# EdoardoLuciani/ARayTracingJourney

Measured on AMD Instinct MI355X. Metric: Mray/s (primary+shadow), Sponza-class 1080p, higher is better.
Workload: dtype f32; 1 GPU; sponza_like(seed=0x5A0A, 262816 triangles, 25 primitives) 1920x1080, 1 light(s), 794216 shadow rays/frame; width=1920, height=1080, lights=1, parallelism=single GPU, 8 frames in flight

## Files before the change

araytracingjourney_amd/csrc/art_trace.hip:

```cpp
#include "art_internal.h"
#include <type_traits>

namespace art {

struct V3 { float x, y, z; };
__device__ __forceinline__ V3 mk(float x, float y, float z) { V3 r; r.x = x; r.y = y; r.z = z; return r; }
__device__ __forceinline__ V3 operator+(V3 a, V3 b) { return mk(a.x + b.x, a.y + b.y, a.z + b.z); }
__device__ __forceinline__ V3 operator-(V3 a, V3 b) { return mk(a.x - b.x, a.y - b.y, a.z - b.z); }
__device__ __forceinline__ V3 operator*(V3 a, V3 b) { return mk(a.x * b.x, a.y * b.y, a.z * b.z); }
__device__ __forceinline__ V3 operator*(V3 a, float s) { return mk(a.x * s, a.y * s, a.z * s); }
__device__ __forceinline__ V3 neg(V3 a) { return mk(-a.x, -a.y, -a.z); }
__device__ __forceinline__ float dot3(V3 a, V3 b) { return fmaf(a.z, b.z, fmaf(a.y, b.y, a.x * b.x)); }
__device__ __forceinline__ V3 cross3(V3 a, V3 b) {
    return mk(fmaf(a.y, b.z, -(a.z * b.y)), fmaf(a.z, b.x, -(a.x * b.z)), fmaf(a.x, b.y, -(a.y * b.x)));
}
constexpr float kExactLo = 0x1p-96f, kExactHi = 0x1p96f;
__device__ __forceinline__ float sqrt_core(float x) {
    float s = __builtin_amdgcn_sqrtf(x);
    float dn = __uint_as_float(__float_as_uint(s) - 1u), up = __uint_as_float(__float_as_uint(s) + 1u);
    float vp = fmaf(-dn, s, x), vs = fmaf(-up, s, x);
    s = vp <= 0.0f ? dn : s;
    return vs > 0.0f ? up : s;
}
__device__ __forceinline__ float rcp_core(float d) {
// ... 128 lines not shown
    float tf = fminf(fminf(fmaxf(t0x, t1x), fmaxf(t0y, t1y)), fmaxf(t0z, t1z));
    return fmaxf(tn, r.tmin) <= fminf(tf, tlimit);
}
#define ART_BARY_EPS 1.0e-6f
__device__ __forceinline__ bool moller_trumbore(const Ray &r, V3 v0, V3 e1, V3 e2, float &t, float &u, float &v) {
    V3 p = cross3(r.d, e2);
    float det = dot3(e1, p);
    if (det == 0.0f) return false;
    float inv = 1.0f / det;
    V3 tv = r.o - v0;
    float uu = dot3(tv, p) * inv;
    if (!(uu >= -ART_BARY_EPS && uu <= 1.0f + ART_BARY_EPS)) return false;
    V3 q = cross3(tv, e1);
    float vv = dot3(r.d, q) * inv;
    if (!(vv >= -ART_BARY_EPS && uu + vv <= 1.0f + ART_BARY_EPS)) return false;
    float tt = dot3(e2, q) * inv;
    if (!(tt > r.tmin && tt < r.tmax)) return false;
    t = tt; u = uu; v = vv;
    return true;
}

__device__ __forceinline__ bool moller_trumbore_flat(const Ray &r, V3 v0, V3 e1, V3 e2, float &t, float &u, float &v) {
    V3 p = cross3(r.d, e2);
    float det = dot3(e1, p);
    float inv = 1.0f / det;
    V3 tv = r.o - v0;
    u = dot3(tv, p) * inv;
    V3 q = cross3(tv, e1);
    v = dot3(r.d, q) * inv;
    t = dot3(e2, q) * inv;
    return (det != 0.0f) & (u >= -ART_BARY_EPS) & (u <= 1.0f + ART_BARY_EPS) & (v >= -ART_BARY_EPS) & (u + v <= 1.0f + ART_BARY_EPS) & (t > r.tmin) & (t < r.tmax);
}

constexpr int kLdsStack = 16;
constexpr int kOvfStack = 80;
constexpr int kBlock = 256;
constexpr int kFrameBlock = 64;
constexpr int kTraceBlock = 64;
struct Tune { uint32_t chunk, refill, blocks, leaf_batch; };
static const Tune kPreset[4] = {{64, 12, 1536, 1}, {128, 24, 1024, 1}, {256, 16, 2048, 8}, {1024, 24, 2048, 8}};
static Tune tune_over(Tune t, const TraceTune &o) {
    if (o.chunk >= 64 && o.chunk <= 65536) t.chunk = o.chunk;
    if (o.refill >= 1 && o.refill <= 64) t.refill = o.refill;
    if (o.blocks >= 1 && o.blocks <= 16384) t.blocks = o.blocks;
    if (o.leaf_batch >= 1 && o.leaf_batch <= 64) t.leaf_batch = o.leaf_batch;
    return t;
}
static Tune tune(bool pipelined, bool ao, const TraceTune &o) { return tune_over(kPreset[(ao ? 2 : 0) + (pipelined ? 1 : 0)], o); }
constexpr int kCursorStride = 32;

__device__ __forceinline__ bool local_to_xy(uint32_t p, const uint32_t *__restrict__ tile_list, uint32_t tiles_x, uint32_t W, uint32_t H, uint32_t &x, uint32_t &y) {
    uint32_t tile = tile_list[p >> 10];
    uint32_t q = p & 1023u, sub = q >> 6, l = q & 63u;
    x = (tile % tiles_x) * kTile + (sub & 3u) * 8u + (l & 7u);
    y = (tile / tiles_x) * kTile + (sub >> 2) * 8u + (l >> 3);
    return x < W && y < H;
}

constexpr int kOvfStack4 = 288;
template <bool ANY, int OVF, int LDSN = kLdsStack, bool ALPHA = false> struct TravBase {
    Ray r;
    float tbest, bu, bv;
    uint32_t bpos, bgid;
    int cur, sp;
    __device__ __forceinline__ void start(V3 o, V3 d, float tmin, float tmax) {
        ray_init(r, o, d, tmin, tmax);
// ... 68 lines not shown
        const bool ngx = r.inv.x < 0.0f, ngy = r.inv.y < 0.0f, ngz = r.inv.z < 0.0f;
        const uint32_t nxw = ngx ? b.w : b.x, fxw = ngx ? b.x : b.w, nyw = ngy ? c.x : b.y, fyw = ngy ? b.y : c.x, nzw = ngz ? c.y : b.z, fzw = ngz ? b.z : c.y;
        const float lim = this->tbest;
#pragma unroll
        for (int i = 0; i < 4; i++) {
            float tnx = fmaf(fmaf((float)((nxw >> (8 * i)) & 255u), sx, ox), r.inv.x, -r.ood.x), tfx = fmaf(fmaf((float)((fxw >> (8 * i)) & 255u), sx, ox), r.inv.x, -r.ood.x);
            float tny = fmaf(fmaf((float)((nyw >> (8 * i)) & 255u), sy, oy), r.inv.y, -r.ood.y), tfy = fmaf(fmaf((float)((fyw >> (8 * i)) & 255u), sy, oy), r.inv.y, -r.ood.y);
            float tnz = fmaf(fmaf((float)((nzw >> (8 * i)) & 255u), sz, oz), r.inv.z, -r.ood.z), tfz = fmaf(fmaf((float)((fzw >> (8 * i)) & 255u), sz, oz), r.inv.z, -r.ood.z);
            float tn = fmaxf(fmaxf(tnx, tny), tnz), tf = fminf(fminf(tfx, tfy), tfz);
            te[i] = tn;
            h[i] = fmaxf(tn, r.tmin) <= fminf(tf, lim);
        }
        float tn = 3.0e38f; int ni = -1;
        if (ANY) {
#pragma unroll
            for (int i = 3; i >= 0; i--) if (h[i]) ni = i;
        } else
#pragma unroll
        for (int i = 0; i < 4; i++) if (h[i] && te[i] < tn) { tn = te[i]; ni = i; }
        if (ni < 0) return this->pop(lds, ovf);
#pragma unroll
        for (int i = 0; i < 4; i++) if (h[i] && i != ni) this->push(refs[i], lds, ovf);
        this->cur = ni == 0 ? refs[0] : (ni == 1 ? refs[1] : (ni == 2 ? refs[2] : refs[3]));
        return false;
    }
};

constexpr int kPacketStack = 288;
__device__ __forceinline__ bool ao_slot_decode(uint32_t slot, uint32_t spp, uint32_t &p, uint32_t &j);
__device__ __forceinline__ V3 ao_dir(V3 N, float tx, float ty, float tz);

__device__ __forceinline__ void ao_ray(const CameraArg &cam, uint32_t W, uint32_t H, uint32_t x, uint32_t y, float depth, float4 nm, uint32_t smp, V3 &o, V3 &d);

__device__ __forceinline__ uint64_t ballot64(bool p) { return __builtin_amdgcn_ballot_w64(p); }

typedef float f4v __attribute__((ext_vector_type(4)));
__device__ __forceinline__ void st_nt(float4 *p, float4 v) { __builtin_nontemporal_store(f4v{v.x, v.y, v.z, v.w}, reinterpret_cast<f4v *>(p)); }
__device__ __forceinline__ void st_nt(float *p, float v) { __builtin_nontemporal_store(v, p); }
typedef float f3v __attribute__((ext_vector_type(3)));
__device__ __forceinline__ void st_nt_rgb(float4 *tiles, size_t texel, float4 v) { __builtin_nontemporal_store(f3v{v.x, v.y, v.z}, reinterpret_cast<f3v *>(reinterpret_cast<float *>(tiles) + 3 * texel)); }
__device__ __forceinline__ float4 ld_nt(const float4 *p) { f4v v = __builtin_nontemporal_load(reinterpret_cast<const f4v *>(p)); return make_float4(v.x, v.y, v.z, v.w); }

template <int OCT> __device__ __forceinline__ bool slab_oct(const Ray &r, float lx, float ly, float lz, float hx, float hy, float hz, float tlimit, float &tn) {
    if (OCT >= 8) return slab(r, lx, ly, lz, hx, hy, hz, tlimit, tn);
    float nx = fmaf((OCT & 1) ? hx : lx, r.inv.x, -r.ood.x), fx = fmaf((OCT & 1) ? lx : hx, r.inv.x, -r.ood.x);
    float ny = fmaf((OCT & 2) ? hy : ly, r.inv.y, -r.ood.y), fy = fmaf((OCT & 2) ? ly : hy, r.inv.y, -r.ood.y);
    float nz = fmaf((OCT & 4) ? hz : lz, r.inv.z, -r.ood.z), fz = fmaf((OCT & 4) ? lz : hz, r.inv.z, -r.ood.z);
    tn = fmaxf(fmaxf(nx, ny), nz);
    float tf = fminf(fminf(fx, fy), fz);
    return fmaxf(tn, r.tmin) <= fminf(tf, tlimit);
}

struct ConstQuads {
    typedef float Quad __attribute__((ext_vector_type(4)));
    __attribute__((address_space(4))) const Quad *p;
    __device__ __forceinline__ float4 operator[](int i) const { Quad v = p[i]; return make_float4(v.x, v.y, v.z, v.w); }
};
template <class T> __device__ __forceinline__ ConstQuads const_quads(const T *p) { ConstQuads q; q.p = (__attribute__((address_space(4))) const ConstQuads::Quad *)(uintptr_t)p; return q; }

#ifdef ART_PACKET_PROF
__device__ unsigned long long g_packet_prof[24];
#define PPROF(i, n) do { if ((threadIdx.x & 63u) == 0) atomicAdd(&g_packet_prof[(ANY ? 12 : 0) + (i)], (unsigned long long)(n)); } while (0)
#else
#define PPROF(i, n)
#endif
struct PacketHints { int cur, sp; uint32_t n; };
__device__ __forceinline__ PacketHints hints_seed(int *stk, uint32_t w0, uint32_t w1, uint32_t w2, uint32_t w3, uint32_t n_leaves) {
    PacketHints h{0, 0, 0u};
    if ((w0 & w1 & w2 & w3) == kHintEmpty) return h;
    const bool lane0 = (threadIdx.x & 63u) == 0;
    if (w3 < n_leaves) { if (lane0) stk[h.sp] = h.cur; h.sp++; h.cur = (int)~w3; }
    if (w2 < n_leaves) { if (lane0) stk[h.sp] = h.cur; h.sp++; h.cur = (int)~w2; }
    if (w1 < n_leaves) { if (lane0) stk[h.sp] = h.cur; h.sp++; h.cur = (int)~w1; }
    if (w0 < n_leaves) { if (lane0) stk[h.sp] = h.cur; h.sp++; h.cur = (int)~w0; }
    return h;
}
template <bool ANY, bool WIDE, int OCT, bool COUNT = false, bool ALPHA = false, bool HINTS = false>
__device__ __forceinline__ void packet_walk(const FrameArgs &a, const Ray &r, bool &on, int *stk, float &tbest, float &bu, float &bv, uint32_t &bpos, uint32_t &bgid, uint32_t &steps, PacketHints &h) {
    int cur = HINTS ? h.cur : 0, sp = HINTS ? h.sp : 0;
    constexpr int kPop = kAbsentChild;
    const auto cull = [&]() -> uint32_t { return ANY ? (a.ray_masks >> 8) & 0xFFu : a.ray_masks & 0xFFu; };
    if (ALPHA && cull() == 0u) return;
#ifdef ART_PACKET_PROF
    unsigned long long pp_[12] = {1, 0, 0, 0, 0, 0, 0, OCT == 8, 0, 0, 0, 0}; bool from_stack_ = false; int hints_left_ = 0;
#endif
#ifdef ART_PACKET_PROF
    if (HINTS) hints_left_ = sp;
#endif
    for (;;) {
#ifdef ART_PACKET_PROF
        const unsigned long long tk0_ = __builtin_amdgcn_s_memtime(); const bool was_node_ = cur >= 0;
#endif
        if (COUNT) steps++;
        if (cur >= 0 && WIDE) {
            ConstQuads nq = const_quads(a.widef + cur);
            float4 w0 = nq[0], w1 = nq[1], w2 = nq[2], w3 = nq[3], w4 = nq[4], w5 = nq[5], w6 = nq[6], w7 = nq[7];
            const int c0 = __float_as_int(w6.x), c1 = __float_as_int(w6.y), c2 = __float_as_int(w6.z), c3 = __float_as_int(w6.w);
            float te;
            const uint64_t m0 = ballot64(slab_oct<OCT>(r, w0.x, w0.y, w0.z, w0.w, w1.x, w1.y, tbest, te));
            const uint64_t m1 = ballot64(slab_oct<OCT>(r, w1.z, w1.w, w2.x, w2.y, w2.z, w2.w, tbest, te));
            const uint64_t m2 = ballot64(slab_oct<OCT>(r, w3.x, w3.y, w3.z, w3.w, w4.x, w4.y, tbest, te));
            const uint64_t m3 = ballot64(slab_oct<OCT>(r, w4.z, w4.w, w5.x, w5.y, w5.z, w5.w, tbest, te));
#ifdef ART_PACKET_PROF
            pp_[1]++; pp_[6] += (m0 != 0ull) + (m1 != 0ull) + (m2 != 0ull) + (m3 != 0ull); from_stack_ = false;
#endif
            const uint32_t ax = __float_as_uint(w7.y);
            const bool rev = OCT < 8 ? ((OCT >> ax) & 1) != 0 : 2 * (int)__popcll(ballot64(on && (ax == 0 ? r.inv.x : (ax == 1 ? r.inv.y : r.inv.z)) < 0.0f)) > (int)__popcll(ballot64(on));
            const bool lane0 = (threadIdx.x & 63u) == 0;
            int next = kPop;
            if (!rev) {
                if (m3 != 0ull) next = c3;
                if (m2 != 0ull) { if (next != kPop) { if (lane0) stk[min(sp, kPacketStack - 1)] = next; sp = min(sp + 1, kPacketStack); } next = c2; }
                if (m1 != 0ull) { if (next != kPop) { if (lane0) stk[min(sp, kPacketStack - 1)] = next; sp = min(sp + 1, kPacketStack); } next = c1; }
                if (m0 != 0ull) { if (next != kPop) { if (lane0) stk[min(sp, kPacketStack - 1)] = next; sp = min(sp + 1, kPacketStack); } next = c0; }
            } else {
                if (m0 != 0ull) next = c0;
                if (m1 != 0ull) { if (next != kPop) { if (lane0) stk[min(sp, kPacketStack - 1)] = next; sp = min(sp + 1, kPacketStack); } next = c1; }
                if (m2 != 0ull) { if (next != kPop) { if (lane0) stk[min(sp, kPacketStack - 1)] = next; sp = min(sp + 1, kPacketStack); } next = c2; }
                if (m3 != 0ull) { if (next != kPop) { if (lane0) stk[min(sp, kPacketStack - 1)] = next; sp = min(sp + 1, kPacketStack); } next = c3; }
            }
            cur = next;
        } else if (cur >= 0) {
            ConstQuads nq = const_quads(a.nodes + cur);
            float4 q0 = nq[0], q1 = nq[1], q2 = nq[2], q3 = nq[3];
            int c0 = __float_as_int(q3.x), c1 = __float_as_int(q3.y);
            float te0, te1;
            uint64_t m0 = ballot64(slab_oct<OCT>(r, q0.x, q0.y, q0.z, q0.w, q1.x, q1.y, tbest, te0));
            uint64_t m1 = ballot64(slab_oct<OCT>(r, q1.z, q1.w, q2.x, q2.y, q2.z, q2.w, tbest, te1));
            if (m0 != 0ull && m1 != 0ull) {
                uint64_t fl = ballot64(te0 <= te1), both = m0 & m1;
                uint64_t f0 = (m0 & ~m1) | (both & fl), f1 = (m1 & ~m0) | (both & ~fl);
                bool first0 = (int)__popcll(f0) >= (int)__popcll(f1);
                if ((threadIdx.x & 63u) == 0) stk[min(sp, kPacketStack - 1)] = first0 ? c1 : c0;
                sp = min(sp + 1, kPacketStack);
                cur = first0 ? c0 : c1;
            } else if (m0 != 0ull) cur = c0;
            else if (m1 != 0ull) cur = c1;
            else cur = kPop;
        } else {
            uint32_t pos = (uint32_t)~cur;
            typedef __attribute__((address_space(4))) const uint32_t *Words;
            bool unseen = false;
            const auto flagged = [&]() -> bool { return ((((Words)(uintptr_t)a.alpha_bits)[pos >> 5] >> (pos & 31u)) & 1u) != 0u; };
            if (ALPHA && flagged()) {
                const float4 s8 = const_quads(a.shade_tris + pos)[8];
                const Words P = (Words)(uintptr_t)(a.prims + __float_as_uint(s8.z));
                unseen = (prim_vis(P[offsetof(DevPrim, masked) / 4]) & cull()) == 0u;
            }
            if (!unseen) {
                ConstQuads tq = const_quads(a.tris + pos);
                float4 ta = tq[0], tb = tq[1], tc = tq[2], td = tq[3];
                float te = 0.f, t = 0.f, u = 0.f, v = 0.f;
                bool acc = moller_trumbore_flat(r, mk(ta.x, ta.y, ta.z), mk(ta.w, tb.x, tb.y), mk(tb.z, tb.w, tc.x), t, u, v) && on;
                if (acc) acc = slab_oct<OCT>(r, tc.y, tc.z, tc.w, td.x, td.y, td.z, tbest, te);
                const auto alpha_keep = [&](bool cand) -> bool {
                    if (!ALPHA || ballot64(cand) == 0ull || !flagged()) return cand;
                    ConstQuads sq = const_quads(a.shade_tris + pos);
                    const float4 s2 = sq[2], s3 = sq[3], s8 = sq[8];
                    const Words P = (Words)(uintptr_t)(a.prims + __float_as_uint(s8.z));
                    const float c = __uint_as_float(P[offsetof(DevPrim, cutoff) / 4]);
                    if (!(c > 0.0f)) return cand;
                    const uint32_t toff = P[offsetof(DevPrim, texture_offset) / 4], tw = P[offsetof(DevPrim, tw) / 4], th = P[offsetof(DevPrim, th) / 4];
                    if (cand) cand = !(alpha_at(a.tex_pool, toff, tw, th, s2, s3, u, v) < c);
                    return cand;
                };
                if (ANY) {
                    if (ALPHA) acc = alpha_keep(acc);
                    bpos = acc ? pos : bpos; on = on && !acc; tbest = acc ? -1.0f : tbest;
                    if (HINTS && ballot64(acc) != 0ull) { if ((threadIdx.x & 63u) == 0) stk[kPacketStack + (h.n & 3u)] = (int)pos; h.n++; }
                }
                else {
                    float teff;
                    asm("v_max_f32 %0, %1, %2" : "=v"(teff) : "v"(t), "v"(te));
                    uint32_t gid = __float_as_uint(td.w);
                    bool better = acc & ((teff < tbest) | ((teff == tbest) & (gid < bgid)));
                    if (ALPHA) better = alpha_keep(better);
                    tbest = better ? teff : tbest; bu = better ? u : bu; bv = better ? v : bv; bpos = better ? pos : bpos; bgid = better ? gid : bgid;
                }
#ifdef ART_PACKET_PROF
                { uint64_t am_ = ballot64(acc); pp_[2]++; pp_[3] += from_stack_; pp_[4] += am_ != 0ull; pp_[5] += __popcll(am_); }
                if (ANY && hints_left_ > 0) { pp_[10]++; pp_[11] += ballot64(on) == 0ull; hints_left_--; }
#endif
                if (ANY && ballot64(on) == 0ull) break;
            }
            cur = kPop;
        }
        if (cur == kPop) {
            if (sp == 0) break;
            sp--;
            cur = __builtin_amdgcn_readfirstlane(stk[sp]);
#ifdef ART_PACKET_PROF
            from_stack_ = true;
#endif
        }
#ifdef ART_PACKET_PROF
        pp_[was_node_ ? 8 : 9] += __builtin_amdgcn_s_memtime() - tk0_;
#endif
    }
#ifdef ART_PACKET_PROF
    for (int i = 0; i < 12; i++) PPROF(i, pp_[i]);
#endif
}

template <bool ANY, bool WIDE, bool COUNT = false, bool ALPHA = false, bool HINTS = false>
__device__ __forceinline__ void walk_dispatch(const FrameArgs &a, const Ray &r, bool &on, int *stk, float &tbest, float &bu, float &bv, uint32_t &bpos, uint32_t &bgid, uint32_t &steps, PacketHints &h) {
    uint64_t act = ballot64(on);
    if (act == 0ull) return;
    uint64_t nx = ballot64(on && r.inv.x < 0.0f), ny = ballot64(on && r.inv.y < 0.0f), nz = ballot64(on && r.inv.z < 0.0f);
    bool uniform = (nx == 0ull || nx == act) && (ny == 0ull || ny == act) && (nz == 0ull || nz == act);
    int oct = !uniform ? 8 : (nx ? 1 : 0) | (ny ? 2 : 0) | (nz ? 4 : 0);
    switch (oct) {
    case 0: packet_walk<ANY, WIDE, 0, COUNT, ALPHA, HINTS>(a, r, on, stk, tbest, bu, bv, bpos, bgid, steps, h); break;
    case 1: packet_walk<ANY, WIDE, 1, COUNT, ALPHA, HINTS>(a, r, on, stk, tbest, bu, bv, bpos, bgid, steps, h); break;
    case 2: packet_walk<ANY, WIDE, 2, COUNT, ALPHA, HINTS>(a, r, on, stk, tbest, bu, bv, bpos, bgid, steps, h); break;
    case 3: packet_walk<ANY, WIDE, 3, COUNT, ALPHA, HINTS>(a, r, on, stk, tbest, bu, bv, bpos, bgid, steps, h); break;
    case 4: packet_walk<ANY, WIDE, 4, COUNT, ALPHA, HINTS>(a, r, on, stk, tbest, bu, bv, bpos, bgid, steps, h); break;
    case 5: packet_walk<ANY, WIDE, 5, COUNT, ALPHA, HINTS>(a, r, on, stk, tbest, bu, bv, bpos, bgid, steps, h); break;
    case 6: packet_walk<ANY, WIDE, 6, COUNT, ALPHA, HINTS>(a, r, on, stk, tbest, bu, bv, bpos, bgid, steps, h); break;
    case 7: packet_walk<ANY, WIDE, 7, COUNT, ALPHA, HINTS>(a, r, on, stk, tbest, bu, bv, bpos, bgid, steps, h); break;
    default: packet_walk<ANY, WIDE, 8, COUNT, ALPHA, HINTS>(a, r, on, stk, tbest, bu, bv, bpos, bgid, steps, h); break;
    }
}

__device__ __forceinline__ uint32_t hilbert_index(uint32_t x, uint32_t y) {
    uint32_t index = 0;
#pragma unroll
    for (uint32_t lvl = 32; lvl > 0; lvl /= 2) {
        uint32_t rx = (x & lvl) > 0, ry = (y & lvl) > 0;
        index += lvl * lvl * ((3u * rx) ^ ry);
        if (ry == 0) {
            if (rx == 1) { x = 63u - x; y = 63u - y; }
            uint32_t t = x; x = y; y = t;
        }
    }
    return index;
}
__device__ __forceinline__ void sincos_turns(float u, float &c, float &s) {
    float q = u * 4.0f;
    int k = (int)q;
    float x = (q - (float)k) * 1.57079632679489662f, x2 = x * x;
    float sp = fmaf(x2, fmaf(x2, fmaf(x2, fmaf(x2, fmaf(x2, -2.50521083854417188e-8f, 2.75573192239858907e-6f), -1.98412698412698413e-4f), 8.33333333333333333e-3f), -1.66666666666666667e-1f), 1.0f) * x;
    float cp = fmaf(x2, fmaf(x2, fmaf(x2, fmaf(x2, fmaf(x2, fmaf(x2, 2.08767569878680990e-9f, -2.75573192239858907e-7f), 2.48015873015873016e-5f), -1.38888888888888889e-3f), 4.16666666666666667e-2f), -0.5f), 1.0f);
    k &= 3;
// ... 971 lines not shown
    V3 out_normal = mk(0.5f, 0.5f, 0.5f);
    uint32_t sbits = 0;
    if (pos == kNoHit) {
        for (uint32_t i = 0; i < a.n_lights; i++) {
            size_t slot = (size_t)i * a.n_local + p;
            st_nt(&a.contrib[slot], make_float4(0.f, 0.f, 0.f, 0.f));
            st_nt(&a.shadow_rays[2 * slot], make_float4(0.f, 0.f, 0.f, -1.0f));
        }
    } else {
        Surface S;
        shade_surface<true>(a, a.cam, pos, h.y, h.z, S, out_depth, out_normal);
        for (uint32_t i = 0; i < a.n_lights; i++) {
            float4 c4, ro, rd;
            const ArtLight L = frame_light(a, i);
            bool want = shade_light<true>(L, S, a.plain_math, c4, ro, rd);
            size_t slot = (size_t)i * a.n_local + p;
            st_nt(&a.contrib[slot], c4);
            if (want) {
                st_nt(&a.shadow_rays[2 * slot], ro);
                st_nt(&a.shadow_rays[2 * slot + 1], rd);
                if (i < 16) sbits |= 1u << (16 + i);
            } else st_nt(&a.shadow_rays[2 * slot], make_float4(0.f, 0.f, 0.f, -1.0f));
        }
    }
    if (in) {
        st_nt(&a.depth[pix], out_depth);
        st_nt(&a.normal[pix], make_float4(out_normal.x, out_normal.y, out_normal.z, 1.0f));
    }
    if (a.shadow_bits) a.shadow_bits[p] = sbits;
    uint64_t hitmask = __ballot(pos != kNoHit);
    if ((threadIdx.x & 63u) == 0 && hitmask) atomicAdd(&a.counters[kHitSlots + ((blockIdx.x * 4u + (threadIdx.x >> 6)) % kSlotCount) * kSlotStride], (uint32_t)__popcll(hitmask));
}

__device__ __forceinline__ uint32_t launder(uint32_t v) { asm volatile("" : "+s"(v)); return v; }
__device__ __forceinline__ uint32_t launder_v(uint32_t v) { asm volatile("" : "+v"(v)); return v; }
__device__ __forceinline__ bool frame_pixel(const FrameArgs &a, uint32_t wid, uint32_t &p, uint32_t &x, uint32_t &y, bool &mine) {
    typedef uint32_t U2 __attribute__((ext_vector_type(2)));
    const U2 item_ = ((__attribute__((address_space(4))) const U2 *)(uintptr_t)a.wave_items)[wid];
    const uint2 item = make_uint2(item_.x, item_.y);
    const uint32_t txy = ((__attribute__((address_space(4))) const uint32_t *)(uintptr_t)a.tile_xy)[item.x >> 4];
    const uint32_t lane = __lane_id(), sub = item.x & 15u;
    p = item.x * 64u + lane;
    mine = (item.y >> (((lane >> 4) << 2) | ((lane >> 1) & 3u))) & 1u;
    x = (txy & 0xFFFFu) * kTile + (sub & 3u) * 8u + (lane & 7u);
    y = (txy >> 16) * kTile + (sub >> 2) * 8u + (lane >> 3);
    return x < a.W && y < a.H && mine;
}
#ifdef ART_PHASE_PROF
constexpr uint32_t kPhaseWaves = 1u << 18;
__device__ uint32_t g_phase[8][kPhaseWaves];
__device__ __forceinline__ uint64_t tick(float &dep) { uint64_t t; asm volatile("s_memtime %0\n\ts_waitcnt lgkmcnt(0)" : "=s"(t), "+v"(dep)); return t; }
#define PHASE(i, dep) { uint64_t t1_ = tick(dep); if (__lane_id() == 0 && blockIdx.x < kPhaseWaves) g_phase[i][blockIdx.x] = (uint32_t)(t1_ - t0_); t0_ = t1_; }
#else
#define PHASE(i, dep)
#endif
template <bool WIDE, bool ONE_LIGHT, bool COUNT, bool BATCH, bool ALPHA> constexpr bool kFrameHints = !(!WIDE && BATCH) && !(ALPHA && !ONE_LIGHT && !COUNT && !BATCH) &&
                                                                                                      !(ALPHA && !WIDE && !ONE_LIGHT && COUNT && !BATCH);
template <bool WIDE, bool ONE_LIGHT, bool COUNT, bool BATCH, bool ALPHA> constexpr bool kFrameFastMath = ONE_LIGHT && !BATCH && !ALPHA;
template <bool WIDE, bool ONE_LIGHT, bool COUNT = false, bool BATCH = false, bool ALPHA = false>
__global__ __launch_bounds__(kFrameBlock) __attribute__((amdgpu_waves_per_eu(8, 8))) void k_frame(FrameArgs a) {
    __shared__ int wstack[kPacketStack + 4];
    constexpr bool HINTS = kFrameHints<WIDE, ONE_LIGHT, COUNT, BATCH, ALPHA>;
    constexpr bool FASTM = kFrameFastMath<WIDE, ONE_LIGHT, COUNT, BATCH, ALPHA>;
    int *stk = wstack;
    const uint32_t wid = blockIdx.x;
    if (wid >= a.n_wave_items) return;
    uint32_t steps = 0;
    const uint32_t fb = BATCH ? blockIdx.y : 0u;
    const CameraArg &cam = (BATCH && fb) ? a.cam_more[fb - 1] : a.cam;
    const size_t frame_px = (size_t)fb * a.W * a.H, frame_local = (size_t)fb * a.n_local;
    bool in;
    Ray r;
#ifdef ART_PHASE_PROF
    float dep0_ = 0.f; uint64_t t0_ = tick(dep0_);
#endif
    {
        uint32_t p, x, y; bool mine;
        in = frame_pixel(a, wid, p, x, y, mine);
        float fx = (float)x + 0.5f, fy = (float)y + 0.5f;
        float dx = (fx / (float)a.W) * 2.0f - 1.0f, dy = (fy / (float)a.H) * 2.0f - 1.0f;
        V3 org = mat4_mul(cam.view_inv, 0.f, 0.f, 0.f, 1.f);
        V3 tgt = nrm3<FASTM>(mat4_mul(cam.proj_inv, dx, dy, 1.f, 1.f), a.plain_math);
        V3 dir = mat4_mul(cam.view_inv, tgt.x, tgt.y, tgt.z, 0.f);
        ray_init(r, org, dir, 0.001f, 10000.0f);
    }
    bool on = in && ray_finite(r.o, r.d);
    PHASE(0, r.inv.x)
    float tbest = on ? r.tmax : -1.0f, bu = 0.f, bv = 0.f;
    uint32_t bpos = kNoHit, bgid = kNoHit;
    { PacketHints none{0, 0, 0u}; walk_dispatch<false, WIDE, COUNT, ALPHA>(a, r, on, stk, tbest, bu, bv, bpos, bgid, steps, none); }
    PHASE(1, tbest)
    uint32_t p, x, y; bool mine;
    frame_pixel(a, wid, p, x, y, mine);
    if (a.keep_hits && mine) a.hits[frame_local + p] = bpos != kNoHit ? make_float4(tbest, bu, bv, __uint_as_float(bpos)) : make_float4(10000.0f, 0.f, 0.f, __uint_as_float(kNoHit));
    const bool hit = in && bpos != kNoHit;
    float out_depth = 10000.0f;
    V3 out_normal = mk(0.5f, 0.5f, 0.5f);
    Surface S;
    S.world_pos = mk(0.f, 0.f, 0.f); S.N = mk(0.f, 0.f, 1.f); S.Vv = mk(0.f, 0.f, 1.f); S.albedo = mk(0.f, 0.f, 0.f);
    S.metallic = 0.f; S.alpha = 0.f; S.nc_NdotV = 0.f; S.NdotV = 0.f;
    if (hit) shade_surface<FASTM, ONE_LIGHT && !BATCH && ALPHA>(a, cam, bpos, bu, bv, S, out_depth, out_normal);
    if (in) {
        const size_t pix = frame_px + (size_t)y * a.W + x;
        st_nt(&a.depth[pix], out_depth);
        st_nt(&a.normal[pix], make_float4(out_normal.x, out_normal.y, out_normal.z, 1.0f));
    }
    PHASE(2, S.NdotV)
    float rx = 0.f, ry = 0.f, rz = 0.f;
    uint32_t sbits = 0, more = 0;
    for (uint32_t i = 0; i < (ONE_LIGHT ? 1u : a.n_lights); i++) {
        PacketHints hn{0, 0, 0u};
        typedef uint32_t U4 __attribute__((ext_vector_type(4)));
        if (HINTS && a.hints) {
            const uint32_t blk = ((__attribute__((address_space(4))) const uint32_t *)(uintptr_t)a.wave_items)[2u * wid];
            const U4 e = ((__attribute__((address_space(4))) const U4 *)(uintptr_t)a.hints)[blk * kHintLights + (i & (kHintLights - 1u))];
            hn = hints_seed(stk, e.x, e.y, e.z, e.w, a.hint_leaves);
        }
        float4 c4 = make_float4(0.f, 0.f, 0.f, 0.f), ro = make_float4(0.f, 0.f, 0.f, 1.0f), rd = make_float4(0.f, 0.f, 1.f, 0.f);
        bool want = false;
        const ArtLight L = ONE_LIGHT ? a.lights[0] : frame_light(a, i);
        if (hit) want = shade_light<FASTM>(L, S, a.plain_math, c4, ro, rd);
        if (want) { if (i < 16u) sbits |= 1u << (16u + i); else more++; }
        Ray sr;
        if (L.type == 2u) ray_init_inv(sr, mk(ro.x, ro.y, ro.z), ld3(L.area_pos2), ld3(L.area_pos3), 0.01f, L.penumbra_angle);
        else ray_init(sr, mk(ro.x, ro.y, ro.z), mk(rd.x, rd.y, rd.z), 0.01f, ro.w);
        bool son = want && ray_finite(sr.o, sr.d);
        PHASE(3, sr.inv.x)
        float st = son ? sr.tmax : -1.0f, su = 0.f, sv = 0.f;
        uint32_t spos = kNoHit, sgid = kNoHit;
        const uint64_t traced = HINTS ? ballot64(son) : 0ull;
        walk_dispatch<true, WIDE, COUNT, ALPHA, HINTS>(a, sr, son, stk, st, su, sv, spos, sgid, steps, hn);
        if (HINTS && a.hints && traced != 0ull) {
            uint32_t o[4];
#pragma unroll
            for (uint32_t k = 0; k < 4u; k++) o[k] = k < hn.n ? (uint32_t)stk[kPacketStack + ((hn.n - 1u - k) & 3u)] : kHintEmpty;
            const uint32_t blk = ((__attribute__((address_space(4))) const uint32_t *)(uintptr_t)a.wave_items)[2u * launder(wid)];
            const size_t at = blk * kHintLights + (i & (kHintLights - 1u));
            const U4 e = ((__attribute__((address_space(4))) const U4 *)(uintptr_t)a.hints)[at];
            if (((e.x ^ o[0]) | (e.y ^ o[1]) | (e.z ^ o[2]) | (e.w ^ o[3])) != 0u && __lane_id() == 0) reinterpret_cast<uint4 *>(a.hints)[at] = make_uint4(o[0], o[1], o[2], o[3]);
        }
        PHASE(4, st)
        if (want && spos != kNoHit) {
            c4 = make_float4(c4.x * 0.05f, c4.y * 0.05f, c4.z * 0.05f, c4.w);
            if (i < 16u) sbits |= 1u << i;
        }
        rx += c4.x * c4.w; ry += c4.y * c4.w; rz += c4.z * c4.w;
    }
    if (!in) { rx = 0.f; ry = 0.f; rz = 0.f; }
    float4 o = make_float4(rx, ry, rz, 1.0f);
    frame_pixel(a, wid, p, x, y, mine);
    if (in) st_nt(&a.color[frame_px + (size_t)y * a.W + x], o);
    if (a.color_tiles && mine) {
        uint32_t q = p & 1023u, sub = q >> 6, l = q & 63u;
        uint32_t lx = (sub & 3u) * 8u + (l & 7u), ly = (sub >> 2) * 8u + (l >> 3);
        size_t ti = (size_t)fb * a.tiles_stride + (size_t)(p >> 10) * kTilePixels + ly * kTile + lx;
        if (a.tiles_packed) __builtin_nontemporal_store(pack_b10g11r11(o.x, o.y, o.z), reinterpret_cast<uint32_t *>(a.color_tiles) + ti);
        else st_nt_rgb(a.color_tiles, ti, o);
    }
    if (mine) a.pix_bits[frame_local + p] = sbits;
    if (!ONE_LIGHT && a.pix_more && mine) a.pix_more[frame_local + p] = more;
    PHASE(5, rx)
#ifdef ART_PHASE_PROF
    if (__lane_id() == 0 && blockIdx.x < kPhaseWaves) { g_phase[6][blockIdx.x] = 1u; g_phase[7][blockIdx.x] = steps; }
#endif
    if (COUNT && __lane_id() == 0) a.wave_cost[wid] = steps;
}

__device__ __forceinline__ uint32_t plan_block_sum(uint32_t v, uint32_t *sh) {
    for (int off = 32; off >= 1; off >>= 1) v += (uint32_t)__shfl_xor((int)v, off);
    __syncthreads();
    if ((threadIdx.x & 63u) == 0) sh[threadIdx.x >> 6] = v;
    __syncthreads();
    uint32_t t = 0;
    for (int i = 0; i < 16; i++) t += sh[i];
    return t;
}
__device__ __forceinline__ uint32_t plan_deal(uint32_t j, uint32_t total) { const uint32_t g = j >> 5; return (g + 1u) * 32u <= total ? g * 32u + 8u * (j & 3u) + ((j & 31u) >> 2) : j; }
__global__ __launch_bounds__(1024) void k_plan(PlanArgs p) {
    __shared__ uint32_t sh[16], sc2[1024], sc1[1024];
    __shared__ unsigned long long sh64[16];
    const uint32_t tid = threadIdx.x;
    unsigned long long sum = 0;
    for (uint32_t i = tid; i < p.n_items_in; i += 1024u) { const uint2 it = p.items_in[i]; if (it.y) { const uint32_t c = p.cost[i]; atomicMax(&p.worst[it.x], c); sum += c; } }
    for (int off = 32; off >= 1; off >>= 1) sum += (unsigned long long)__shfl_xor((long long)sum, off);
    if ((tid & 63u) == 0) sh64[tid >> 6] = sum;
    __threadfence_block();
    __syncthreads();
    sum = 0;
    for (int i = 0; i < 16; i++) sum += sh64[i];
    uint32_t T = p.fixed_steps ? p.fixed_steps : max(p.min_steps, (uint32_t)(p.share * (float)sum));
    const uint32_t per = (p.n64 + 1023u) / 1024u, b0 = min(tid * per, p.n64), b1 = min(b0 + per, p.n64);
    uint32_t n1 = 0, n2 = 0, N1 = 0, N2 = 0, ups = 0, downs = 0, split = 0, wmax = 0;
    for (int attempt = 0; attempt < 8; attempt++, T += T / 2) {
        n1 = n2 = 0; uint32_t u = 0, d = 0, sp = 0;
        for (uint32_t b = b0; b < b1; b++) {
            const uint32_t w = __hip_atomic_load(&p.worst[b], __ATOMIC_RELAXED, __HIP_MEMORY_SCOPE_AGENT);
            const uint32_t old = p.level[b];
            uint32_t lv = old;
// ... 353 lines not shown
```

Measured before the change: 23020 Mray/s.

## Track packet lane activity as scalar wave masks and rematerialize kernel args

The packet BVH walk can now carry the active-lane set as a 64-bit scalar ballot mask instead of a per-lane bool. Triangle test results become ballots, and hit-record updates are deferred to a single masked v_cndmask select after each step, which moves predicate work onto the scalar unit and reduces VGPR pressure. A per-variant table also chooses whether k_frame re-reads FrameArgs from the kernarg segment at several points, so argument values need not stay live in registers across traversal. The cost is more inline asm and template complexity, and the register-allocation and scheduling effects are hard to predict.

```diff
diff --git a/araytracingjourney_amd/csrc/art_trace.hip b/araytracingjourney_amd/csrc/art_trace.hip
--- a/araytracingjourney_amd/csrc/art_trace.hip
+++ b/araytracingjourney_amd/csrc/art_trace.hip
@@ -184,6 +184,20 @@
     return (det != 0.0f) & (u >= -ART_BARY_EPS) & (u <= 1.0f + ART_BARY_EPS) & (v >= -ART_BARY_EPS) & (u + v <= 1.0f + ART_BARY_EPS) & (t > r.tmin) & (t < r.tmax);
 }
 
+__device__ __forceinline__ uint64_t moller_trumbore_mask(const Ray &r, V3 v0, V3 e1, V3 e2, float &t, float &u, float &v) {
+    V3 p = cross3(r.d, e2);
+    float det = dot3(e1, p);
+    float inv = 1.0f / det;
+    V3 tv = r.o - v0;
+    u = dot3(tv, p) * inv;
+    V3 q = cross3(tv, e1);
+    v = dot3(r.d, q) * inv;
+    t = dot3(e2, q) * inv;
+    return __builtin_amdgcn_ballot_w64(det != 0.0f) & __builtin_amdgcn_ballot_w64(u >= -ART_BARY_EPS) & __builtin_amdgcn_ballot_w64(u <= 1.0f + ART_BARY_EPS) &
+           __builtin_amdgcn_ballot_w64(v >= -ART_BARY_EPS) & __builtin_amdgcn_ballot_w64(u + v <= 1.0f + ART_BARY_EPS) & __builtin_amdgcn_ballot_w64(t > r.tmin) &
+           __builtin_amdgcn_ballot_w64(t < r.tmax);
+}
+
 constexpr int kLdsStack = 16;
 constexpr int kOvfStack = 80;
 constexpr int kBlock = 256;
@@ -318,7 +332,12 @@
 
 __device__ __forceinline__ void ao_ray(const CameraArg &cam, uint32_t W, uint32_t H, uint32_t x, uint32_t y, float depth, float4 nm, uint32_t smp, V3 &o, V3 &d);
 
+__device__ __forceinline__ uint32_t launder(uint32_t v) { asm volatile("" : "+s"(v)); return v; }
+__device__ __forceinline__ uint32_t launder_v(uint32_t v) { asm volatile("" : "+v"(v)); return v; }
 __device__ __forceinline__ uint64_t ballot64(bool p) { return __builtin_amdgcn_ballot_w64(p); }
+__device__ __forceinline__ void sel(float &x, float y, uint64_t m) { asm("v_cndmask_b32_e64 %0, %0, %1, %2" : "+v"(x) : "v"(y), "s"(m)); }
+__device__ __forceinline__ void sel(uint32_t &x, uint32_t y, uint64_t m) { asm("v_cndmask_b32_e64 %0, %0, %1, %2" : "+v"(x) : "v"(y), "s"(m)); }
+__device__ __forceinline__ void sel_off(float &x, uint64_t m) { asm("v_cndmask_b32_e64 %0, %0, -1.0, %1" : "+v"(x) : "s"(m)); }
 
 typedef float f4v __attribute__((ext_vector_type(4)));
 __device__ __forceinline__ void st_nt(float4 *p, float4 v) { __builtin_nontemporal_store(f4v{v.x, v.y, v.z, v.w}, reinterpret_cast<f4v *>(p)); }
@@ -361,8 +380,11 @@
     if (w0 < n_leaves) { if (lane0) stk[h.sp] = h.cur; h.sp++; h.cur = (int)~w0; }
     return h;
 }
-template <bool ANY, bool WIDE, int OCT, bool COUNT = false, bool ALPHA = false, bool HINTS = false>
-__device__ __forceinline__ void packet_walk(const FrameArgs &a, const Ray &r, bool &on, int *stk, float &tbest, float &bu, float &bv, uint32_t &bpos, uint32_t &bgid, uint32_t &steps, PacketHints &h) {
+struct StepUpdate { uint64_t m = 0ull; float t, u, v; uint32_t pos, gid; };
+struct NoUpdate {};
+template <bool ANY, bool WIDE, int OCT, bool COUNT = false, bool ALPHA = false, bool HINTS = false, class ON>
+__device__ __forceinline__ void packet_walk(const FrameArgs &a, const Ray &r, ON &on, int *stk, float &tbest, float &bu, float &bv, uint32_t &bpos, uint32_t &bgid, uint32_t &steps, PacketHints &h) {
+    constexpr bool MASKS = std::is_same<ON, uint64_t>::value;
     int cur = HINTS ? h.cur : 0, sp = HINTS ? h.sp : 0;
     constexpr int kPop = kAbsentChild;
     const auto cull = [&]() -> uint32_t { return ANY ? (a.ray_masks >> 8) & 0xFFu : a.ray_masks & 0xFFu; };
@@ -373,10 +395,12 @@
 #ifdef ART_PACKET_PROF
     if (HINTS) hints_left_ = sp;
 #endif
+    typename std::conditional<MASKS, StepUpdate, NoUpdate>::type up;
     for (;;) {
 #ifdef ART_PACKET_PROF
         const unsigned long long tk0_ = __builtin_amdgcn_s_memtime(); const bool was_node_ = cur >= 0;
 #endif
+        if constexpr (MASKS) up.m = 0ull;
         if (COUNT) steps++;
         if (cur >= 0 && WIDE) {
             ConstQuads nq = const_quads(a.widef + cur);
@@ -391,7 +415,9 @@
             pp_[1]++; pp_[6] += (m0 != 0ull) + (m1 != 0ull) + (m2 != 0ull) + (m3 != 0ull); from_stack_ = false;
 #endif
             const uint32_t ax = __float_as_uint(w7.y);
-            const bool rev = OCT < 8 ? ((OCT >> ax) & 1) != 0 : 2 * (int)__popcll(ballot64(on && (ax == 0 ? r.inv.x : (ax == 1 ? r.inv.y : r.inv.z)) < 0.0f)) > (int)__popcll(ballot64(on));
+            bool rev = ((OCT >> ax) & 1) != 0;
+            if constexpr (OCT >= 8 && MASKS) rev = 2 * (int)__popcll(on & ballot64((ax == 0 ? r.inv.x : (ax == 1 ? r.inv.y : r.inv.z)) < 0.0f)) > (int)__popcll(on);
+            else if constexpr (OCT >= 8) rev = 2 * (int)__popcll(ballot64(on && (ax == 0 ? r.inv.x : (ax == 1 ? r.inv.y : r.inv.z)) < 0.0f)) > (int)__popcll(ballot64(on));
             const bool lane0 = (threadIdx.x & 63u) == 0;
             int next = kPop;
             if (!rev) {
@@ -437,39 +463,77 @@
                 ConstQuads tq = const_quads(a.tris + pos);
                 float4 ta = tq[0], tb = tq[1], tc = tq[2], td = tq[3];
                 float te = 0.f, t = 0.f, u = 0.f, v = 0.f;
-                bool acc = moller_trumbore_flat(r, mk(ta.x, ta.y, ta.z), mk(ta.w, tb.x, tb.y), mk(tb.z, tb.w, tc.x), t, u, v) && on;
-                if (acc) acc = slab_oct<OCT>(r, tc.y, tc.z, tc.w, td.x, td.y, td.z, tbest, te);
-                const auto alpha_keep = [&](bool cand) -> bool {
-                    if (!ALPHA || ballot64(cand) == 0ull || !flagged()) return cand;
-                    ConstQuads sq = const_quads(a.shade_tris + pos);
-                    const float4 s2 = sq[2], s3 = sq[3], s8 = sq[8];
-                    const Words P = (Words)(uintptr_t)(a.prims + __float_as_uint(s8.z));
-                    const float c = __uint_as_float(P[offsetof(DevPrim, cutoff) / 4]);
-                    if (!(c > 0.0f)) return cand;
-                    const uint32_t toff = P[offsetof(DevPrim, texture_offset) / 4], tw = P[offsetof(DevPrim, tw) / 4], th = P[offsetof(DevPrim, th) / 4];
-                    if (cand) cand = !(alpha_at(a.tex_pool, toff, tw, th, s2, s3, u, v) < c);
-                    return cand;
-                };
-                if (ANY) {
-                    if (ALPHA) acc = alpha_keep(acc);
-                    bpos = acc ? pos : bpos; on = on && !acc; tbest = acc ? -1.0f : tbest;
-                    if (HINTS && ballot64(acc) != 0ull) { if ((threadIdx.x & 63u) == 0) stk[kPacketStack + (h.n & 3u)] = (int)pos; h.n++; }
+                if constexpr (MASKS) {
+                    uint64_t acc = moller_trumbore_mask(r, mk(ta.x, ta.y, ta.z), mk(ta.w, tb.x, tb.y), mk(tb.z, tb.w, tc.x), t, u, v) & on;
+                    if (acc != 0ull) acc &= ballot64(slab_oct<OCT>(r, tc.y, tc.z, tc.w, td.x, td.y, td.z, tbest, te));
+                    const auto alpha_keep = [&](uint64_t cand) -> uint64_t {
+                        if (!ALPHA || cand == 0ull || !flagged()) return cand;
+                        ConstQuads sq = const_quads(a.shade_tris + pos);
+                        const float4 s2 = sq[2], s3 = sq[3], s8 = sq[8];
+                        const Words P = (Words)(uintptr_t)(a.prims + __float_as_uint(s8.z));
+                        const float c = __uint_as_float(P[offsetof(DevPrim, cutoff) / 4]);
+                        if (!(c > 0.0f)) return cand;
+                        const uint32_t toff = P[offsetof(DevPrim, texture_offset) / 4], tw = P[offsetof(DevPrim, tw) / 4], th = P[offsetof(DevPrim, th) / 4];
+                        bool keep = __builtin_amdgcn_inverse_ballot_w64(cand);
+                        if (keep) keep = !(alpha_at(a.tex_pool, toff, tw, th, s2, s3, u, v) < c);
+                        return cand & ballot64(keep);
+                    };
+                    if (ANY) {
+                        if (ALPHA) acc = alpha_keep(acc);
+                        up.m = acc; up.pos = pos; on &= ~acc;
+                        if (HINTS && acc != 0ull) { const uint32_t n = launder(h.n); if ((threadIdx.x & 63u) == 0) stk[kPacketStack + (n & 3u)] = (int)pos; h.n = n + 1u; }
+                    }
+                    else {
+                        float teff;
+                        asm("v_max_f32 %0, %1, %2" : "=v"(teff) : "v"(t), "v"(te));
+                        uint32_t gid = __float_as_uint(td.w);
+                        uint64_t better = acc & (ballot64(teff < tbest) | (ballot64(teff == tbest) & ballot64(gid < bgid)));
+                        if (ALPHA) better = alpha_keep(better);
+                        up.m = better; up.t = teff; up.u = u; up.v = v; up.pos = pos; up.gid = gid;
+                    }
+#ifdef ART_PACKET_PROF
+                    { uint64_t am_ = acc; pp_[2]++; pp_[3] += from_stack_; pp_[4] += am_ != 0ull; pp_[5] += __popcll(am_); }
+                    if (ANY && hints_left_ > 0) { pp_[10]++; pp_[11] += on == 0ull; hints_left_--; }
+#endif
+                } else {
+                    bool acc = moller_trumbore_flat(r, mk(ta.x, ta.y, ta.z), mk(ta.w, tb.x, tb.y), mk(tb.z, tb.w, tc.x), t, u, v) && on;
+                    if (acc) acc = slab_oct<OCT>(r, tc.y, tc.z, tc.w, td.x, td.y, td.z, tbest, te);
+                    const auto alpha_keep = [&](bool cand) -> bool {
+                        if (!ALPHA || ballot64(cand) == 0ull || !flagged()) return cand;
+                        ConstQuads sq = const_quads(a.shade_tris + pos);
+                        const float4 s2 = sq[2], s3 = sq[3], s8 = sq[8];
+                        const Words P = (Words)(uintptr_t)(a.prims + __float_as_uint(s8.z));
+                        const float c = __uint_as_float(P[offsetof(DevPrim, cutoff) / 4]);
+                        if (!(c > 0.0f)) return cand;
+                        const uint32_t toff = P[offsetof(DevPrim, texture_offset) / 4], tw = P[offsetof(DevPrim, tw) / 4], th = P[offsetof(DevPrim, th) / 4];
+                        if (cand) cand = !(alpha_at(a.tex_pool, toff, tw, th, s2, s3, u, v) < c);
+                        return cand;
+                    };
+                    if (ANY) {
+                        if (ALPHA) acc = alpha_keep(acc);
+                        bpos = acc ? pos : bpos; on = on && !acc; tbest = acc ? -1.0f : tbest;
+                        if (HINTS && ballot64(acc) != 0ull) { if ((threadIdx.x & 63u) == 0) stk[kPacketStack + (h.n & 3u)] = (int)pos; h.n++; }
+                    }
+                    else {
+                        float teff;
+                        asm("v_max_f32 %0, %1, %2" : "=v"(teff) : "v"(t), "v"(te));
+                        uint32_t gid = __float_as_uint(td.w);
+                        bool better = acc & ((teff < tbest) | ((teff == tbest) & (gid < bgid)));
+                        if (ALPHA) better = alpha_keep(better);
+                        tbest = better ? teff : tbest; bu = better ? u : bu; bv = better ? v : bv; bpos = better ? pos : bpos; bgid = better ? gid : bgid;
+                    }
+#ifdef ART_PACKET_PROF
+                    { uint64_t am_ = ballot64(acc); pp_[2]++; pp_[3] += from_stack_; pp_[4] += am_ != 0ull; pp_[5] += __popcll(am_); }
+                    if (ANY && hints_left_ > 0) { pp_[10]++; pp_[11] += ballot64(on) == 0ull; hints_left_--; }
+#endif
                 }
-                else {
-                    float teff;
-                    asm("v_max_f32 %0, %1, %2" : "=v"(teff) : "v"(t), "v"(te));
-                    uint32_t gid = __float_as_uint(td.w);
-                    bool better = acc & ((teff < tbest) | ((teff == tbest) & (gid < bgid)));
-                    if (ALPHA) better = alpha_keep(better);
-                    tbest = better ? teff : tbest; bu = better ? u : bu; bv = better ? v : bv; bpos = better ? pos : bpos; bgid = better ? gid : bgid;
-                }
-#ifdef ART_PACKET_PROF
-                { uint64_t am_ = ballot64(acc); pp_[2]++; pp_[3] += from_stack_; pp_[4] += am_ != 0ull; pp_[5] += __popcll(am_); }
-                if (ANY && hints_left_ > 0) { pp_[10]++; pp_[11] += ballot64(on) == 0ull; hints_left_--; }
-#endif
-                if (ANY && ballot64(on) == 0ull) break;
+                if constexpr (!MASKS) { if (ANY && ballot64(on) == 0ull) break; }
             }
             cur = kPop;
+        }
+        if constexpr (MASKS) if (up.m != 0ull) {
+            if (ANY) { sel(bpos, up.pos, up.m); sel_off(tbest, up.m); if (on == 0ull) break; }
+            else { sel(tbest, up.t, up.m); sel(bu, up.u, up.m); sel(bv, up.v, up.m); sel(bpos, up.pos, up.m); sel(bgid, up.gid, up.m); }
         }
         if (cur == kPop) {
             if (sp == 0) break;
@@ -488,13 +552,25 @@
 #endif
 }
 
-template <bool ANY, bool WIDE, bool COUNT = false, bool ALPHA = false, bool HINTS = false>
-__device__ __forceinline__ void walk_dispatch(const FrameArgs &a, const Ray &r, bool &on, int *stk, float &tbest, float &bu, float &bv, uint32_t &bpos, uint32_t &bgid, uint32_t &steps, PacketHints &h) {
-    uint64_t act = ballot64(on);
-    if (act == 0ull) return;
-    uint64_t nx = ballot64(on && r.inv.x < 0.0f), ny = ballot64(on && r.inv.y < 0.0f), nz = ballot64(on && r.inv.z < 0.0f);
-    bool uniform = (nx == 0ull || nx == act) && (ny == 0ull || ny == act) && (nz == 0ull || nz == act);
-    int oct = !uniform ? 8 : (nx ? 1 : 0) | (ny ? 2 : 0) | (nz ? 4 : 0);
+template <bool ANY, bool WIDE, bool COUNT = false, bool ALPHA = false, bool HINTS = false, bool MASKS = true>
+__device__ __forceinline__ void walk_dispatch(const FrameArgs &a, const Ray &r, bool alive, int *stk, float &tbest, float &bu, float &bv, uint32_t &bpos, uint32_t &bgid, uint32_t &steps, PacketHints &h) {
+    typename std::conditional<MASKS, uint64_t, bool>::type on;
+    int oct;
+    if constexpr (MASKS) {
+        on = ballot64(alive);
+        const uint64_t act = on;
+        if (act == 0ull) return;
+        uint64_t nx = act & ballot64(r.inv.x < 0.0f), ny = act & ballot64(r.inv.y < 0.0f), nz = act & ballot64(r.inv.z < 0.0f);
+        bool uniform = (nx == 0ull || nx == act) && (ny == 0ull || ny == act) && (nz == 0ull || nz == act);
+        oct = !uniform ? 8 : (int)(launder(nx ? 2u : 0u) >> 1) | (ny ? 2 : 0) | (nz ? 4 : 0);
+    } else {
+        on = alive;
+        uint64_t act = ballot64(on);
+        if (act == 0ull) return;
+        uint64_t nx = ballot64(on && r.inv.x < 0.0f), ny = ballot64(on && r.inv.y < 0.0f), nz = ballot64(on && r.inv.z < 0.0f);
+        bool uniform = (nx == 0ull || nx == act) && (ny == 0ull || ny == act) && (nz == 0ull || nz == act);
+        oct = !uniform ? 8 : (nx ? 1 : 0) | (ny ? 2 : 0) | (nz ? 4 : 0);
+    }
     switch (oct) {
     case 0: packet_walk<ANY, WIDE, 0, COUNT, ALPHA, HINTS>(a, r, on, stk, tbest, bu, bv, bpos, bgid, steps, h); break;
     case 1: packet_walk<ANY, WIDE, 1, COUNT, ALPHA, HINTS>(a, r, on, stk, tbest, bu, bv, bpos, bgid, steps, h); break;
@@ -1532,8 +1608,6 @@
     if ((threadIdx.x & 63u) == 0 && hitmask) atomicAdd(&a.counters[kHitSlots + ((blockIdx.x * 4u + (threadIdx.x >> 6)) % kSlotCount) * kSlotStride], (uint32_t)__popcll(hitmask));
 }
 
-__device__ __forceinline__ uint32_t launder(uint32_t v) { asm volatile("" : "+s"(v)); return v; }
-__device__ __forceinline__ uint32_t launder_v(uint32_t v) { asm volatile("" : "+v"(v)); return v; }
 __device__ __forceinline__ bool frame_pixel(const FrameArgs &a, uint32_t wid, uint32_t &p, uint32_t &x, uint32_t &y, bool &mine) {
     typedef uint32_t U2 __attribute__((ext_vector_type(2)));
     const U2 item_ = ((__attribute__((address_space(4))) const U2 *)(uintptr_t)a.wave_items)[wid];
@@ -1557,18 +1631,34 @@
 template <bool WIDE, bool ONE_LIGHT, bool COUNT, bool BATCH, bool ALPHA> constexpr bool kFrameHints = !(!WIDE && BATCH) && !(ALPHA && !ONE_LIGHT && !COUNT && !BATCH) &&
                                                                                                       !(ALPHA && !WIDE && !ONE_LIGHT && COUNT && !BATCH);
 template <bool WIDE, bool ONE_LIGHT, bool COUNT, bool BATCH, bool ALPHA> constexpr bool kFrameFastMath = ONE_LIGHT && !BATCH && !ALPHA;
+constexpr uint8_t kFrameMovesTable[32] = {55, 63, 63, 63, 55, 63, 0, 0, 49, 55, 63, 0, 49, 63, 63, 56, 31, 63, 63, 0, 63, 63, 63, 63, 19, 63, 0, 0, 19, 63, 0, 0};
+#ifdef ART_MOVES_FORCE
+template <bool WIDE, bool ONE_LIGHT, bool COUNT, bool BATCH, bool ALPHA> constexpr uint32_t kFrameMoves = ART_MOVES_FORCE;
+#else
+template <bool WIDE, bool ONE_LIGHT, bool COUNT, bool BATCH, bool ALPHA> constexpr uint32_t kFrameMoves = kFrameMovesTable[WIDE << 4 | ONE_LIGHT << 3 | COUNT << 2 | BATCH << 1 | ALPHA];
+#endif
+__device__ __forceinline__ const FrameArgs &frame_args_again(const FrameArgs &a) {
+#ifdef __HIP_DEVICE_COMPILE__
+    __attribute__((address_space(4))) const char *p = (__attribute__((address_space(4))) const char *)__builtin_amdgcn_kernarg_segment_ptr();
+    asm volatile("" : "+s"(p));
+    return *(const FrameArgs *)p;
+#else
+    return a;
+#endif
+}
 template <bool WIDE, bool ONE_LIGHT, bool COUNT = false, bool BATCH = false, bool ALPHA = false>
-__global__ __launch_bounds__(kFrameBlock) __attribute__((amdgpu_waves_per_eu(8, 8))) void k_frame(FrameArgs a) {
+__global__ __launch_bounds__(kFrameBlock) __attribute__((amdgpu_waves_per_eu(8, 8))) void k_frame(FrameArgs a_) {
     __shared__ int wstack[kPacketStack + 4];
     constexpr bool HINTS = kFrameHints<WIDE, ONE_LIGHT, COUNT, BATCH, ALPHA>;
     constexpr bool FASTM = kFrameFastMath<WIDE, ONE_LIGHT, COUNT, BATCH, ALPHA>;
+    constexpr uint32_t MV = kFrameMoves<WIDE, ONE_LIGHT, COUNT, BATCH, ALPHA>;
     int *stk = wstack;
     const uint32_t wid = blockIdx.x;
-    if (wid >= a.n_wave_items) return;
+    if (wid >= a_.n_wave_items) return;
     uint32_t steps = 0;
     const uint32_t fb = BATCH ? blockIdx.y : 0u;
-    const CameraArg &cam = (BATCH && fb) ? a.cam_more[fb - 1] : a.cam;
-    const size_t frame_px = (size_t)fb * a.W * a.H, frame_local = (size_t)fb * a.n_local;
+    const CameraArg &cam0 = (BATCH && fb) ? a_.cam_more[fb - 1] : a_.cam;
+    const size_t frame_px = (size_t)fb * a_.W * a_.H, frame_local = (size_t)fb * a_.n_local;
     bool in;
     Ray r;
 #ifdef ART_PHASE_PROF
@@ -1576,20 +1666,23 @@
 #endif
     {
         uint32_t p, x, y; bool mine;
-        in = frame_pixel(a, wid, p, x, y, mine);
+        in = frame_pixel(a_, wid, p, x, y, mine);
         float fx = (float)x + 0.5f, fy = (float)y + 0.5f;
-        float dx = (fx / (float)a.W) * 2.0f - 1.0f, dy = (fy / (float)a.H) * 2.0f - 1.0f;
-        V3 org = mat4_mul(cam.view_inv, 0.f, 0.f, 0.f, 1.f);
-        V3 tgt = nrm3<FASTM>(mat4_mul(cam.proj_inv, dx, dy, 1.f, 1.f), a.plain_math);
-        V3 dir = mat4_mul(cam.view_inv, tgt.x, tgt.y, tgt.z, 0.f);
+        float dx = (fx / (float)a_.W) * 2.0f - 1.0f, dy = (fy / (float)a_.H) * 2.0f - 1.0f;
+        V3 org = mat4_mul(cam0.view_inv, 0.f, 0.f, 0.f, 1.f);
+        V3 tgt = nrm3<FASTM>(mat4_mul(cam0.proj_inv, dx, dy, 1.f, 1.f), a_.plain_math);
+        V3 dir = mat4_mul(cam0.view_inv, tgt.x, tgt.y, tgt.z, 0.f);
         ray_init(r, org, dir, 0.001f, 10000.0f);
     }
     bool on = in && ray_finite(r.o, r.d);
     PHASE(0, r.inv.x)
     float tbest = on ? r.tmax : -1.0f, bu = 0.f, bv = 0.f;
     uint32_t bpos = kNoHit, bgid = kNoHit;
-    { PacketHints none{0, 0, 0u}; walk_dispatch<false, WIDE, COUNT, ALPHA>(a, r, on, stk, tbest, bu, bv, bpos, bgid, steps, none); }
+    { PacketHints none{0, 0, 0u}; walk_dispatch<false, WIDE, COUNT, ALPHA, false, (MV & 1u) != 0u>(a_, r, on, stk, tbest, bu, bv, bpos, bgid, steps, none); }
     PHASE(1, tbest)
+    const FrameArgs &a = (MV & 2u) ? frame_args_again(a_) : a_;
+    const FrameArgs &as = (MV & 4u) ? a : a_;
+    const CameraArg &cam = (BATCH && fb) ? as.cam_more[fb - 1] : as.cam;
     uint32_t p, x, y; bool mine;
     frame_pixel(a, wid, p, x, y, mine);
     if (a.keep_hits && mine) a.hits[frame_local + p] = bpos != kNoHit ? make_float4(tbest, bu, bv, __uint_as_float(bpos)) : make_float4(10000.0f, 0.f, 0.f, __uint_as_float(kNoHit));
@@ -1599,7 +1692,7 @@
     Surface S;
     S.world_pos = mk(0.f, 0.f, 0.f); S.N = mk(0.f, 0.f, 1.f); S.Vv = mk(0.f, 0.f, 1.f); S.albedo = mk(0.f, 0.f, 0.f);
     S.metallic = 0.f; S.alpha = 0.f; S.nc_NdotV = 0.f; S.NdotV = 0.f;
-    if (hit) shade_surface<FASTM, ONE_LIGHT && !BATCH && ALPHA>(a, cam, bpos, bu, bv, S, out_depth, out_normal);
+    if (hit) shade_surface<FASTM, ONE_LIGHT && !BATCH && ALPHA>(as, cam, bpos, bu, bv, S, out_depth, out_normal);
     if (in) {
         const size_t pix = frame_px + (size_t)y * a.W + x;
         st_nt(&a.depth[pix], out_depth);
@@ -1608,18 +1701,19 @@
     PHASE(2, S.NdotV)
     float rx = 0.f, ry = 0.f, rz = 0.f;
     uint32_t sbits = 0, more = 0;
-    for (uint32_t i = 0; i < (ONE_LIGHT ? 1u : a.n_lights); i++) {
+    for (uint32_t i = 0; i < (ONE_LIGHT ? 1u : a_.n_lights); i++) {
+        const FrameArgs &b = (MV & 8u) ? frame_args_again(a_) : a_;
         PacketHints hn{0, 0, 0u};
         typedef uint32_t U4 __attribute__((ext_vector_type(4)));
-        if (HINTS && a.hints) {
-            const uint32_t blk = ((__attribute__((address_space(4))) const uint32_t *)(uintptr_t)a.wave_items)[2u * wid];
-            const U4 e = ((__attribute__((address_space(4))) const U4 *)(uintptr_t)a.hints)[blk * kHintLights + (i & (kHintLights - 1u))];
-            hn = hints_seed(stk, e.x, e.y, e.z, e.w, a.hint_leaves);
+        if (HINTS && b.hints) {
+            const uint32_t blk = ((__attribute__((address_space(4))) const uint32_t *)(uintptr_t)b.wave_items)[2u * wid];
+            const U4 e = ((__attribute__((address_space(4))) const U4 *)(uintptr_t)b.hints)[blk * kHintLights + (i & (kHintLights - 1u))];
+            hn = hints_seed(stk, e.x, e.y, e.z, e.w, b.hint_leaves);
         }
         float4 c4 = make_float4(0.f, 0.f, 0.f, 0.f), ro = make_float4(0.f, 0.f, 0.f, 1.0f), rd = make_float4(0.f, 0.f, 1.f, 0.f);
         bool want = false;
-        const ArtLight L = ONE_LIGHT ? a.lights[0] : frame_light(a, i);
-        if (hit) want = shade_light<FASTM>(L, S, a.plain_math, c4, ro, rd);
+        const ArtLight L = ONE_LIGHT ? b.lights[0] : frame_light(b, i);
+        if (hit) want = shade_light<FASTM>(L, S, b.plain_math, c4, ro, rd);
         if (want) { if (i < 16u) sbits |= 1u << (16u + i); else more++; }
         Ray sr;
         if (L.type == 2u) ray_init_inv(sr, mk(ro.x, ro.y, ro.z), ld3(L.area_pos2), ld3(L.area_pos3), 0.01f, L.penumbra_angle);
@@ -1629,15 +1723,16 @@
         float st = son ? sr.tmax : -1.0f, su = 0.f, sv = 0.f;
         uint32_t spos = kNoHit, sgid = kNoHit;
         const uint64_t traced = HINTS ? ballot64(son) : 0ull;
-        walk_dispatch<true, WIDE, COUNT, ALPHA, HINTS>(a, sr, son, stk, st, su, sv, spos, sgid, steps, hn);
-        if (HINTS && a.hints && traced != 0ull) {
+        walk_dispatch<true, WIDE, COUNT, ALPHA, HINTS, (MV & 1u) != 0u>(b, sr, son, stk, st, su, sv, spos, sgid, steps, hn);
+        const FrameArgs &c = (MV & 16u) ? frame_args_again(a_) : a_;
+        if (HINTS && c.hints && traced != 0ull) {
             uint32_t o[4];
 #pragma unroll
             for (uint32_t k = 0; k < 4u; k++) o[k] = k < hn.n ? (uint32_t)stk[kPacketStack + ((hn.n - 1u - k) & 3u)] : kHintEmpty;
-            const uint32_t blk = ((__attribute__((address_space(4))) const uint32_t *)(uintptr_t)a.wave_items)[2u * launder(wid)];
+            const uint32_t blk = ((__attribute__((address_space(4))) const uint32_t *)(uintptr_t)c.wave_items)[2u * launder(wid)];
             const size_t at = blk * kHintLights + (i & (kHintLights - 1u));
-            const U4 e = ((__attribute__((address_space(4))) const U4 *)(uintptr_t)a.hints)[at];
-            if (((e.x ^ o[0]) | (e.y ^ o[1]) | (e.z ^ o[2]) | (e.w ^ o[3])) != 0u && __lane_id() == 0) reinterpret_cast<uint4 *>(a.hints)[at] = make_uint4(o[0], o[1], o[2], o[3]);
+            const U4 e = ((__attribute__((address_space(4))) const U4 *)(uintptr_t)c.hints)[at];
+            if (((e.x ^ o[0]) | (e.y ^ o[1]) | (e.z ^ o[2]) | (e.w ^ o[3])) != 0u && __lane_id() == 0) reinterpret_cast<uint4 *>(c.hints)[at] = make_uint4(o[0], o[1], o[2], o[3]);
         }
         PHASE(4, st)
         if (want && spos != kNoHit) {
@@ -1648,22 +1743,23 @@
     }
     if (!in) { rx = 0.f; ry = 0.f; rz = 0.f; }
     float4 o = make_float4(rx, ry, rz, 1.0f);
-    frame_pixel(a, wid, p, x, y, mine);
-    if (in) st_nt(&a.color[frame_px + (size_t)y * a.W + x], o);
-    if (a.color_tiles && mine) {
+    const FrameArgs &e = (MV & 32u) ? frame_args_again(a_) : a_;
+    frame_pixel(e, wid, p, x, y, mine);
+    if (in) st_nt(&e.color[frame_px + (size_t)y * e.W + x], o);
+    if (e.color_tiles && mine) {
         uint32_t q = p & 1023u, sub = q >> 6, l = q & 63u;
         uint32_t lx = (sub & 3u) * 8u + (l & 7u), ly = (sub >> 2) * 8u + (l >> 3);
-        size_t ti = (size_t)fb * a.tiles_stride + (size_t)(p >> 10) * kTilePixels + ly * kTile + lx;
-        if (a.tiles_packed) __builtin_nontemporal_store(pack_b10g11r11(o.x, o.y, o.z), reinterpret_cast<uint32_t *>(a.color_tiles) + ti);
-        else st_nt_rgb(a.color_tiles, ti, o);
-    }
-    if (mine) a.pix_bits[frame_local + p] = sbits;
-    if (!ONE_LIGHT && a.pix_more && mine) a.pix_more[frame_local + p] = more;
+        size_t ti = (size_t)fb * e.tiles_stride + (size_t)(p >> 10) * kTilePixels + ly * kTile + lx;
+        if (e.tiles_packed) __builtin_nontemporal_store(pack_b10g11r11(o.x, o.y, o.z), reinterpret_cast<uint32_t *>(e.color_tiles) + ti);
+        else st_nt_rgb(e.color_tiles, ti, o);
+    }
+    if (mine) e.pix_bits[frame_local + p] = sbits;
+    if (!ONE_LIGHT && e.pix_more && mine) e.pix_more[frame_local + p] = more;
     PHASE(5, rx)
 #ifdef ART_PHASE_PROF
     if (__lane_id() == 0 && blockIdx.x < kPhaseWaves) { g_phase[6][blockIdx.x] = 1u; g_phase[7][blockIdx.x] = steps; }
 #endif
-    if (COUNT && __lane_id() == 0) a.wave_cost[wid] = steps;
+    if (COUNT && __lane_id() == 0) e.wave_cost[wid] = steps;
 }
 
 __device__ __forceinline__ uint32_t plan_block_sum(uint32_t v, uint32_t *sh) {
```

Result: faster. 23450 Mray/s (median of 6 runs) (+1.8%).
